# Vanlightly/vsr-tlaplus

Measured on AMD Instinct MI355X. Metric: distinct states/sec (whole node) + time-to-first-violation, VSR 3-replica, higher is better.
Workload: dtype u64

## Files before the change

### vsr_tlaplus_amd/csrc/host_checker.hpp

```cpp
#pragma once

struct PassDst {
  u64* words = nullptr;
  u64 words_cap = 0;
  u64* off = nullptr;
  u64* fp = nullptr;
  u64 cap = 0;
  bool own_words = true;
  bool own_index = true;
};
struct DeepLevelRec { u64 n_new = 0, n_local = 0, generated = 0, max_bag = 0, frontier = 0; };
struct vsrmc_deep_attach;
struct vsrmc_checker {
  vsrmc_model model;
  vsrmc_options opt;
  hipStream_t stream = nullptr;
  hipEvent_t ev[4] = {nullptr, nullptr, nullptr, nullptr};
  Slot* table = nullptr;
  u64 tmask = 0;
  u64* words[2] = {nullptr, nullptr};
  u64* off[2] = {nullptr, nullptr};
  u64* lvl_fp = nullptr;
  u64* pending = nullptr;
  LevelCtl* ctl = nullptr;
// ... 182 lines not shown
    if (hipFuncGetAttributes(&at, c->plain5_kernel) == hipSuccess && dyn + at.sharedSizeBytes <= LDS5_MAX &&
        hipOccupancyMaxActiveBlocksPerMultiprocessor(&nb5, c->plain5_kernel, blk, dyn) == hipSuccess && nb5 >= VSR_OCC + 1) {
      f.kernel = c->plain5_kernel; f.ccap = cc5; f.lds = dyn; f.blocks_per_cu = (unsigned)(VSR_OCC + 1);
    }
  }
  return f;
}

int wset_ensure(vsrmc_checker* c) {
  if (c->opt.world <= 1) return 0;
  if (c->d_wset) {
    if (c->wset_dirty) {
      HIPCHK(hipMemsetAsync(c->h_wset.fp, 0, (c->h_wset.mask + 1) * 8, c->stream));
      HIPCHK(hipMemsetAsync(c->h_wset.epoch, 0, (c->h_wset.mask + 1) * 4, c->stream));
      c->wset_dirty = false;
      c->wepoch = 0;
    }
    return 0;
  }
  u64 slots = std::max<u64>((u64)1 << 12, (c->tmask + 1) / 2);
  while (true) {
    hipError_t e = hipMalloc((void**)&c->h_wset.fp, slots * 8);
    if (e == hipSuccess) e = hipMalloc((void**)&c->h_wset.epoch, slots * 4);
    if (e == hipSuccess) break;
    (void)hipGetLastError();
    if (c->h_wset.fp) (void)hipFree(c->h_wset.fp);
    c->h_wset.fp = nullptr;
    if (slots <= ((u64)1 << 16)) return fail(VSRMC_E_HIP, "hipMalloc of the winner set of the sharded deep search failed");
    slots /= 2;
  }
  c->h_wset.mask = slots - 1;
  HIPCHK(hipMemsetAsync(c->h_wset.fp, 0, slots * 8, c->stream));
  HIPCHK(hipMemsetAsync(c->h_wset.epoch, 0, slots * 4, c->stream));
  HIPCHK(hipMalloc((void**)&c->d_wset, sizeof(WSet)));
  HIPCHK(hipMemcpyAsync(c->d_wset, &c->h_wset, sizeof(WSet), hipMemcpyHostToDevice, c->stream));
  HIPCHK(hipStreamSynchronize(c->stream));
  c->wepoch = 0;
  c->wset_dirty = false;
  return 0;
}
u64 wset_count(const vsrmc_checker* c) {
  u64 n = 0;
  for (const DeepLevelRec& d : c->deep_lv) n += d.n_local;
  return n;
}
int wset_grow(vsrmc_checker* c) {
  if (!c->d_wset) return 1;
  const u64 old_slots = c->h_wset.mask + 1, slots = old_slots * 2;
  u64* nfp = nullptr;
  u32* nep = nullptr;
  u32* d_err = nullptr;
  size_t free_b = 0, total_b = 0;
  if (hipMemGetInfo(&free_b, &total_b) != hipSuccess || (double)slots * 12.0 + 1.0e9 > (double)free_b) return 1;
  bool ok = hipMalloc((void**)&nfp, slots * 8) == hipSuccess && hipMalloc((void**)&nep, slots * 4) == hipSuccess && hipMalloc((void**)&d_err, 4) == hipSuccess;
  ok = ok && hipMemsetAsync(nfp, 0, slots * 8, c->stream) == hipSuccess && hipMemsetAsync(nep, 0, slots * 4, c->stream) == hipSuccess &&
       hipMemsetAsync(d_err, 0, 4, c->stream) == hipSuccess;
  u32 err = 0;
  if (ok) {
    hipLaunchKernelGGL(k_wset_rehash, dim3(4096), dim3(256), 0, c->stream, (const u64*)c->h_wset.fp, (const u32*)c->h_wset.epoch, old_slots, nfp, nep, slots - 1, d_err);
    ok = hipGetLastError() == hipSuccess && hipMemcpyAsync(&err, d_err, 4, hipMemcpyDeviceToHost, c->stream) == hipSuccess && hipStreamSynchronize(c->stream) == hipSuccess && err == 0;
  }
  if (d_err) (void)hipFree(d_err);
  if (!ok) {
    (void)hipGetLastError();
    if (nfp) (void)hipFree(nfp);
    if (nep) (void)hipFree(nep);
    return 1;
  }
  (void)hipFree(c->h_wset.fp);
  (void)hipFree(c->h_wset.epoch);
  c->h_wset.fp = nfp; c->h_wset.epoch = nep; c->h_wset.mask = slots - 1;
  if (hipMemcpy(c->d_wset, &c->h_wset, sizeof(WSet), hipMemcpyHostToDevice) != hipSuccess) return fail(VSRMC_E_HIP, "winner set: descriptor copy");
  return 0;
}
void wset_free(vsrmc_checker* c) {
  if (c->h_wset.fp) (void)hipFree(c->h_wset.fp);
  if (c->h_wset.epoch) (void)hipFree(c->h_wset.epoch);
  if (c->d_wset) (void)hipFree(c->d_wset);
  c->h_wset.fp = nullptr; c->h_wset.epoch = nullptr; c->h_wset.mask = 0; c->d_wset = nullptr; c->wepoch = 0;
}

void deep_free_scratch(vsrmc_checker* c);

int checker_seed(vsrmc_checker* c) {
  const Model& M = c->model.M;
  deep_free_scratch(c);
#ifdef VSRMC_TEST_HOOKS
  c->test_seed_index.clear(); c->test_seed_words.clear(); c->test_seed_off.clear();
#endif
  c->rebase_off = false;
  c->saw_violation = false;
  c->deep = 0;
  c->deep_lv.clear();
  c->deep_g = 2;
  c->deep_distinct = c->deep_generated = 0;
  c->deep_regen_done = false;
  c->hist_new[0] = c->hist_new[1] = 0;
  c->g_last = 16;
  c->cur_rec_w = 0;
  c->failed = 0;
  c->failed_code = 0;
  c->full_recoverable = false;
  HIPCHK(hipSetDevice(c->opt.device));
  if (c->claim_bits) { (void)hipFree(c->claim_bits); c->claim_bits = nullptr; c->claim_w = c->claim_parents = 0; }
  if (c->d_wset && c->wset_used) c->wset_dirty = true;
  c->wset_used = false;
  hipLaunchKernelGGL(k_table_init, dim3(4096), dim3(256), 0, c->stream, c->table, c->tmask + 1);
  HIPCHK(hipGetLastError());
  std::vector<u64> wire, dev(512);
  init_record_wire(M, wire);
  int len = wire_to_device(M, wire.data(), dev.data());
  u64 H[6];
  hash_full_host(M, (const u64*)dev.data(), H);
  for (int i = 0; i < M.np; i++) dev[M.h0 + i] = H[i];
  u64 zero = (u64)len, init_fp = 0;
  u32 init_ak = 0;
  canonical_fp(M, dev[0], &dev[M.h0], &init_fp, &init_ak);
  const bool mine = true;
  if (c->filter) HIPCHK(hipMemsetAsync(c->filter, 0, (c->fmask + 1) * 8, c->stream));
  HIPCHK(hipMemsetAsync(c->ctl, 0, sizeof(LevelCtl), c->stream));
  if (mine) {
    HIPCHK(hipMemcpyAsync(c->words[0], dev.data(), len * 8, hipMemcpyDefault, c->stream));
    HIPCHK(hipMemcpyAsync(c->off[0], &zero, 8, hipMemcpyHostToDevice, c->stream));
    hipLaunchKernelGGL(k_seed, dim3(1), dim3(64), 0, c->stream, M, c->words[0], c->table, c->tmask, c->lvl_fp, c->ctl);
    HIPCHK(hipGetLastError());
  }
  HIPCHK(hipStreamSynchronize(c->stream));
  c->cur = 0;
  c->level = 1;
  c->n_frontier = mine ? 1 : 0;
  c->n_valid = c->n_frontier;
  c->cur_w = (u64)len;
  c->distinct = mine ? 1 : 0;
  c->total_generated = 0;
  c->failed = 0;
  c->cur_max_bag = 0;
  c->bag_known = true;
  c->failed_code = 0;
  c->probe_fp = 0;
  c->probe_level = 0;
  c->probe_extra_fp = 0;
  c->probe_viol.clear();
  c->probe_viol_key.clear();
  c->probe_viol_level = 0;
  deep_attach_restart(c);
  return 0;
}
}

extern "C" {

void vsrmc_options_default(vsrmc_options* o) {
  if (!o) return;
  std::memset(o, 0, sizeof(*o));
  o->device = 0;
  o->table_log2 = 26;
  o->frontier_words = (uint64_t)1 << 27;
  o->frontier_states = (uint64_t)1 << 22;
  o->pending_entries = (uint64_t)1 << 23;
  o->keep_trace = 1;
  o->trace_entries = 0;
  o->rank = 0;
  o->world = 1;
}

static int autosize_options(vsrmc_options* o, const Model& M) {
  if (o->table_log2 != 0 && o->frontier_words != 0) {
    if (o->pending_entries == 0) o->pending_entries = o->exact_ties ? (u64)1 << 24 : (u64)1 << 16;
    if (o->frontier_states == 0) o->frontier_states = std::max<u64>((u64)1 << 16, o->frontier_words / 24);
    return 0;
  }
  size_t free_b = 0, total_b = 0;
  HIPCHK(hipSetDevice(o->device));
  HIPCHK(hipMemGetInfo(&free_b, &total_b));
  const char* share_env = std::getenv("VSRMC_AUTOSIZE_SHARE");
  const double share = share_env ? std::max(1.0, std::atof(share_env)) : 1.0;
  double avail = ((double)free_b - 4.0e9) / share;
  if (avail < 256e6) return fail(VSRMC_E_HIP, "less than 256 MB of free device memory to size the checker from");
  if (o->table_log2 == 0) {
    int lg = 8;
    while (lg < 36 && (double)((u64)1 << (lg + 1)) * 16.0 <= 0.30 * avail) lg++;
    o->table_log2 = lg;
  }
  avail -= (double)((u64)1 << o->table_log2) * 16.0;
  if (o->world > 1 && !o->exact_ties) avail -= (double)((u64)1 << (o->filter_log2 > 0 ? o->filter_log2 : o->table_log2)) * 8.0;
  if (o->world > 1 && !o->exact_ties) avail -= (double)((u64)1 << o->table_log2) * 6.0;
  if (o->pending_entries == 0) o->pending_entries = o->exact_ties ? (u64)1 << 24 : (u64)1 << 16;
// ... 671 lines not shown
```

### vsr_tlaplus_amd/csrc/vsr_deep.hpp

```cpp
#pragma once

namespace {

typedef DeepLevelRec DeepLevel;

struct Slicer {
  u64 cap_n, cap_w, g1, stride;
  u64 cap_c = ~(u64)0;
  double yield_n = 0, yield_w = 0;
  u64 worst() const {
    const u64 sz = std::min<u64>(std::min<u64>(cap_n / (4 * g1), cap_w / (4 * g1 * stride)), cap_c);
    return std::max<u64>(128, sz & ~(u64)127);
  }
  u64 next() const {
    if (yield_n <= 0) return worst();
    const double sz = std::min((double)cap_n / (3.0 * std::max(yield_n, 1e-3)), (double)cap_w / (3.0 * std::max(yield_w, 1e-3)));
    return std::max<u64>(worst(), std::min<u64>(cap_c, std::max<u64>(128, (u64)std::min(sz, 1e15) & ~(u64)127)));
  }
  void expect(double per_n, double per_w) { yield_n = std::max(yield_n, per_n); yield_w = std::max(yield_w, per_w); }
  void observe(u64 n_src, u64 n_out, u64 w_out) {
    if (!n_src) return;
    yield_n = std::max(yield_n, (double)n_out / (double)n_src);
    yield_w = std::max(yield_w, (double)w_out / (double)n_src);
  }
};

struct DeepRun;
struct DeepIo {
  void* ctx = nullptr;
  int world = 1;
  u64 cand_cap = 0;
  int (*pass)(void* ctx, const u64* sw, const u64* so, u64 n, u64 p_off, int level, int mode, u64 bag, const PassDst* dst) = nullptr;
  int (*any)(void* ctx, u64* flag) = nullptr;
  int (*reduce)(void* ctx, DeepRun* R) = nullptr;
  int (*resolve)(void* ctx, DeepRun* R) = nullptr;
};

struct DeepRun {
  vsrmc_checker* c;
  const DeepIo* io = nullptr;
  int base;
  int last_regen;
  bool insert;
  vsrmc_level_info ins, prb;
  u64 viol_ins = ~(u64)0;
  u32 mask_ins = 0, mask_prb = 0;
  std::vector<u64> bad;
  u64 launches = 0, n_slices = 0, n_subs = 0;
  u64* d_sum = nullptr;
  bool rebase = false;
  u64* d_cnt = nullptr;
  u32* d_err = nullptr;
  int err = 0;
  int probed_level() const { return last_regen + (insert ? 2 : 1); }
};

void deep_free_scratch(vsrmc_checker* c) {
  for (PassDst& B : c->scratch) {
    if (B.words && B.own_words) (void)hipFree(B.words);
    if (B.off && B.own_index) (void)hipFree(B.off);
    if (B.fp && B.own_index) (void)hipFree(B.fp);
  }
  c->scratch.clear();
  c->scratch0 = PassDst();
  c->scratch_carved = false;
  c->scratch_buf = -1;
  c->scratch_front = 0;
}

int deep_plan_scratch(vsrmc_checker* c, int count, bool carve = true, u64 front = 0) {
  if (count < 0) count = 0;
  if (count > 400) return fail(VSRMC_E_REP, "deep search: more than 400 nested levels");
  const int nxt = c->cur ^ 1;
  if ((c->host_frontier >> nxt) & 1) carve = false;
  front = (front + 63) & ~(u64)63;
  const bool same_buf = !c->scratch_carved || c->scratch_buf == nxt;
  if ((size_t)count <= c->scratch.size() && c->scratch_front == front && same_buf && (c->scratch_carved == carve || (count == 0 && !carve))) return 0;
  deep_free_scratch(c);
  if (count == 0) return 0;
  size_t free_b = 0, total_b = 0;
  HIPCHK(hipMemGetInfo(&free_b, &total_b));
  const char* share_env = std::getenv("VSRMC_AUTOSIZE_SHARE");
  const double share = share_env ? std::max(1.0, std::atof(share_env)) : 1.0;
  const double reserve = std::max(0.0, (double)free_b - 1.0e9) / share;
  if (front >= c->words_cap(nxt)) carve = false;
  const double idle_w = (double)(c->words_cap(nxt) - (carve ? front : 0));
  const int with0 = front ? 0 : 1;
  const u64 floor_w = (u64)1 << 21;
  const double w_old = std::max((double)floor_w, std::min(idle_w / 4.0, reserve / (double)count / 9.34));
  const double cost_old = (with0 ? 1.0 / idle_w : 0.0) + (double)count / w_old;
  int best_n = 0;
  double best_s = 0;
  if (carve)
    for (int n_idle = 1; n_idle <= count + with0; n_idle++) {
      const double from_res = (double)(count + with0 - n_idle) * 9.34 + (double)(n_idle - with0) * 1.34;
      const double s = std::min(idle_w / (double)n_idle, from_res > 0 ? reserve / from_res : 1e30);
      if (s > best_s) { best_s = s; best_n = n_idle; }
    }
  const bool carved = carve && best_n >= 1 + with0 && best_s >= (double)floor_w && (double)(count + with0) / best_s < cost_old;
  const u64 wcap = carved ? (u64)best_s & ~(u64)63 : (u64)w_old;
  auto alloc_index = [&](PassDst& B) -> bool {
    B.cap = std::max<u64>((u64)1 << 15, B.words_cap / 12);
    return hipMalloc((void**)&B.off, (B.cap + 1) * 8) == hipSuccess && hipMalloc((void**)&B.fp, B.cap * 8) == hipSuccess;
  };
  bool ok = true;
  if (carved && with0) {
    c->scratch0.words = c->words[nxt]; c->scratch0.words_cap = wcap; c->scratch0.own_words = false;
    c->scratch0.off = c->off[nxt]; c->scratch0.fp = c->lvl_fp; c->scratch0.own_index = false;
    c->scratch0.cap = std::min<u64>(c->opt.frontier_states, std::max<u64>((u64)1 << 15, wcap / 12));
  }
  for (int k = 1; k <= count && ok; k++) {
    PassDst B;
    B.words_cap = wcap;
    if (carved && k - 1 + with0 < best_n) { B.words = c->words[nxt] + front + (u64)(k - 1 + with0) * wcap; B.own_words = false; }
    else ok = hipMalloc((void**)&B.words, B.words_cap * 8) == hipSuccess;
    ok = ok && alloc_index(B);
    c->scratch.push_back(B);
  }
  if (!ok) {
    (void)hipGetLastError();
    deep_free_scratch(c);
    return fail(VSRMC_E_HIP, "hipMalloc of a deep-search scratch buffer failed");
  }
  c->scratch_carved = carve;
  c->scratch_buf = nxt;
  c->scratch_front = front;
  return 0;
}

int deep_buffer(vsrmc_checker* c, int k, PassDst* out) {
  const int nxt = c->cur ^ 1;
  if (k == 0) {
// ... 39 lines not shown
  u64 f = (mine ? 1 : 0) | (R.err ? 2 : 0);
  if (R.io) *rc = R.io->any(R.io->ctx, &f);
  if (!*rc && f >= 2) *rc = R.err ? R.err : fail(VSRMC_E_STATE, "deep pass: another rank failed between two exchanges");
  return !*rc && (f & 1) != 0;
}
int deep_local_fail(DeepRun& R, int rc) {
  if (!R.io) return rc;
  if (!R.err) R.err = rc;
  return 0;
}
u64 deep_cand_bound(const DeepRun& R, u64 g1) {
  if (!R.io || R.io->world <= 1) return ~(u64)0;
  return std::max<u64>(128, (u64)(0.45 * (double)R.io->cand_cap * (double)R.io->world / (double)std::max<u64>(1, g1)) & ~(u64)127);
}

int deep_probe(DeepRun& R, const PassDst& B, u64 n, int lv, u64 bag) {
  vsrmc_checker* c = R.c;
  if (!n) return 0;
  c->expand_ms = 0;
  if (R.err) return 0;
  int rc = expand_pass(c, B.words, B.off, n, 0, lv + 1, MODE_PROBE, bag);
  R.launches += c->extra_launches;
  if (!rc && c->h.limit_unchecked) {
    R.prb.limit_rechecked += c->h.limit_unchecked;
    c->probe_all_actions = true;
    rc = expand_pass(c, B.words, B.off, n, 0, lv + 1, MODE_PROBE, bag);
    c->probe_all_actions = false;
    R.launches += 1 + c->extra_launches;
  }
  if (rc) return deep_local_fail(R, rc);
  R.launches++;
  deep_acc(&R.prb, c->h, c->expand_ms);
  if (c->h.n_pending) {
    R.mask_prb |= c->h.viol_mask;
    if (c->h.n_pending > c->opt.pending_entries || R.bad.size() / 2 + c->h.n_pending > ((u64)1 << 24))
      return deep_local_fail(R, fail(VSRMC_E_REP, "more violating successors in the probed level than the pending list holds (pending_entries)"));
    const size_t at = R.bad.size();
    R.bad.resize(at + 2 * c->h.n_pending);
    if (hipMemcpy(R.bad.data() + at, c->pending, 16 * c->h.n_pending, hipMemcpyDeviceToHost) != hipSuccess)
      return deep_local_fail(R, fail(VSRMC_E_HIP, "deep search: copy of the probe's candidates"));
  }
  return 0;
}

int deep_export(DeepRun& R, const PassDst& B, u64 part) {
  vsrmc_checker* c = R.c;
  if (!part) return 0;
  const int nxt = c->cur ^ 1;
  hipLaunchKernelGGL(k_export, dim3((unsigned)((part + 63) / 64)), dim3(64), 0, c->stream, (const u64*)B.words, B.off, B.fp, (u64)0, part,
                     c->words[nxt], c->scratch_front ? c->scratch_front : c->words_cap(nxt), c->off[nxt], c->lvl_fp, c->opt.frontier_states, R.d_cnt, R.d_err);
  if (hipGetLastError() != hipSuccess || hipStreamSynchronize(c->stream) != hipSuccess) return fail(VSRMC_E_HIP, "deep search: k_export (re-basing)");
  return 0;
}

int deep_descend(DeepRun& R, const u64* src_words, const u64* src_off, u64 n_idx, u64 src_bag, int lv, int k) {
  vsrmc_checker* c = R.c;
  const Model& M = c->model.M;
  PassDst B;
  int rc = deep_buffer(c, k, &B);
  if (rc) return rc;
  Slicer sl;
  sl.cap_n = B.cap; sl.cap_w = B.words_cap; sl.g1 = std::max<u64>(1, c->deep_g); sl.stride = (u64)c->lds_stride;
  sl.cap_c = deep_cand_bound(R, sl.g1);
  const bool regen = lv + 1 <= R.last_regen;
  const DeepLevel& next = c->deep_lv[(size_t)(lv - R.base)];
  if (regen) {
    const u64 parents = lv == R.base ? c->n_valid : c->deep_lv[(size_t)(lv - R.base - 1)].n_local;
    const double per_n = (double)next.n_local / (double)std::max<u64>(1, parents);
    const double wbar = (lv == R.base ? (double)c->cur_w / (double)std::max<u64>(1, c->n_valid) : (double)(M.fixed + (int)src_bag)) + 2.0;
    sl.expect(per_n, per_n * wbar);
  }
  const u64 out_bag = regen ? std::min<u64>(next.max_bag, (u64)M.max_bag) : 0;
  for (u64 a = 0; deep_more(R, a < n_idx, &rc);) {
    if (rc) return rc;
    const u64 n = a < n_idx ? std::min<u64>(sl.next(), n_idx - a) : 0;
    c->expand_ms = 0;
    rc = deep_run_pass(R, src_words, src_off + a, n, (R.io && c->opt.world > 1) ? 0 : a, lv + 1, regen ? MODE_REGEN : MODE_NORMAL, src_bag, &B);
    if (rc) return rc;
    if (n) R.launches += 1 + c->extra_launches;
    a += n;
    if (n) (k == 0 ? R.n_slices : R.n_subs)++;
    const u64 part = c->h.n_new;
    sl.observe(n, part, c->h.words_new);
    if (regen) {
      R.ins.materialize_ms += c->expand_ms;
      if (c->deep_attach && !R.io && (rc = deep_where_slice(c, B, part, lv + 1, 0, out_bag, false)) != 0) return rc;
      if (lv + 1 == R.last_regen && !R.insert) rc = R.rebase ? deep_export(R, B, part) : deep_probe(R, B, part, lv + 1, out_bag);
      else rc = deep_descend(R, B.words, B.off, part, out_bag, lv + 1, k + 1);
      if (rc) return rc;
      continue;
    }
    deep_acc(&R.ins, c->h, c->expand_ms);
    R.ins.record_words += c->h.rec_words;
    R.ins.max_bag = std::max<u64>(R.ins.max_bag, c->h.max_bag);
    if (c->h.viol_fp != ~(u64)0) {
      R.mask_ins |= c->h.viol_mask;
      R.viol_ins = std::min<u64>(R.viol_ins, c->h.viol_fp);
    }
    if (!part) continue;
    const u64 bag_new = std::min<u64>(c->h.max_bag, (u64)M.max_bag);
    {
      u64 hsum[3] = {0, 0, 0};
      bool ok = hipMemsetAsync(R.d_sum, 0, 24, c->stream) == hipSuccess;
      if (ok) hipLaunchKernelGGL(k_level_checksum, dim3(1024), dim3(256), 0, c->stream, B.fp, part, R.d_sum);
      ok = ok && hipGetLastError() == hipSuccess && hipMemcpyAsync(hsum, R.d_sum, 24, hipMemcpyDeviceToHost, c->stream) == hipSuccess &&
           hipStreamSynchronize(c->stream) == hipSuccess;
      if (!ok) {
        rc = deep_local_fail(R, fail(VSRMC_E_HIP, "deep search: k_level_checksum"));
        if (rc) return rc;
        continue;
      }
      R.ins.fp_xor ^= hsum[0];
      R.ins.fp_sum += hsum[1];
      R.ins.n_new += hsum[2];
    }
    if (c->deep_attach && !R.io && (rc = deep_where_slice(c, B, part, lv + 1, 1, bag_new, R.viol_ins == ~(u64)0)) != 0) return rc;
    if (R.viol_ins != ~(u64)0) continue;
    rc = deep_probe(R, B, part, lv + 1, bag_new);
    if (rc) return rc;
  }
  return rc;
}

int deep_resolve(DeepRun& R) {
  vsrmc_checker* c = R.c;
  const u64 nbad = R.bad.size() / 2;
  if (!nbad) return 0;
  const int plevel = R.probed_level();
  std::vector<std::pair<u64, u64>> pairs(nbad);
  for (u64 i = 0; i < nbad; i++) pairs[i] = std::make_pair(R.bad[2 * i], R.bad[2 * i + 1]);
  std::sort(pairs.begin(), pairs.end());
  std::vector<u64> fps;
  for (u64 i = 0; i < nbad; i++)
    if (i == 0 || pairs[i].first != pairs[i - 1].first) fps.push_back(pairs[i].first);
  std::vector<uint8_t> seen8(fps.size(), 0);
  int rc = vsrmc_checker_seen_batch(c, fps.data(), (u64)fps.size(), plevel, seen8.data());
  if (rc) return rc;
  u64 first = ~(u64)0, key = ~(u64)0;
  size_t g = 0;
  for (u64 i = 0; i < nbad; i++) {
    if (i && pairs[i].first != pairs[i - 1].first) g++;
    if (seen8[g]) continue;
    R.prb.pending++;
    if (first == ~(u64)0) { first = pairs[i].first; key = pairs[i].second; }
    if (c->probe_viol.empty() || c->probe_viol.back() != pairs[i].first) {
      c->probe_viol.push_back(pairs[i].first);
      c->probe_viol_key.push_back(pairs[i].second);
    }
  }
  c->probe_viol_level = plevel;
  if (first == ~(u64)0) return 0;
  int found = 0;
  u64 pfp = 0, pmeta = 0;
  rc = table_lookup(c, meta_pfp(key), plevel - 1, 1, &found, &pfp, &pmeta);
  if (rc) return rc;
  if (found > 1) return fail(VSRMC_E_STATE, "ambiguous predecessor pointer: several states of the parent's level share the 45 fingerprint bits the violating successor keeps of its parent");
  R.prb.viol_fp = first;
  R.prb.viol_mask = (int32_t)R.mask_prb;
  if (found) { c->probe_fp = pfp; c->probe_level = plevel - 1; c->probe_extra_fp = first; }
  return 0;
}

int deep_check_ready(vsrmc_checker* c, int extra_levels, bool sharded) {
  if (c->opt.exact_ties) return fail(VSRMC_E_STATE, "levels beyond the record buffers need a single-pass checker");
  if (!sharded && c->opt.world > 1) return fail(VSRMC_E_STATE, "a sharded checker goes beyond its record buffers with vsrmc_shard_loop_deepen");
  if (c->failed) return fail(VSRMC_E_STATE, "the checker stopped on an error");
  if (c->level + c->deep + extra_levels >= 511) return fail(VSRMC_E_REP, "more than 510 BFS levels");
  return 0;
}

int deep_first_pass(vsrmc_checker* c, vsrmc_level_info* ins, const DeepIo* io = nullptr) {
  const Model& M = c->model.M;
  DeepRun R;
  R.c = c; R.io = io; R.base = c->level; R.last_regen = c->level; R.insert = true;
  std::memset(&R.ins, 0, sizeof(R.ins));
  std::memset(&R.prb, 0, sizeof(R.prb));
  R.ins.viol_fp = R.ins.viol_index = R.prb.viol_fp = R.prb.viol_index = ~(u64)0;
  const double t0 = now_s();
  const u64 bagL = c->bag_known ? c->cur_max_bag : (u64)M.max_bag;
  c->deep = 1;
  c->deep_lv.assign(1, DeepLevel());
  const u64 cb = deep_cand_bound(R, std::max<u64>(c->deep_g, c->g_last));
  if (!io || c->opt.world == 1) deep_claim_bits_alloc(c, bagL);
  int rc = 0;
  for (u64 a = 0; deep_more(R, a < c->n_frontier, &rc);) {
    if (rc) break;
    const u64 n = a < c->n_frontier ? std::min<u64>(cb, c->n_frontier - a) : 0;
    c->expand_ms = 0;
    rc = deep_run_pass(R, c->words[c->cur], c->off[c->cur] + a, n, (io && c->opt.world > 1) ? 0 : a, c->level + 1, MODE_INSERT, bagL, nullptr);
    if (rc) break;
    a += n;
    if (n) R.launches += 1 + c->extra_launches;
    deep_acc(&R.ins, c->h, c->expand_ms);
    R.ins.n_new += c->h.n_new;
    R.ins.max_bag = std::max<u64>(R.ins.max_bag, c->h.max_bag);
    R.ins.fp_xor ^= c->h.fp_xor;
    R.ins.fp_sum += c->h.fp_sum;
    if (c->h.viol_fp != ~(u64)0) { R.mask_ins |= c->h.viol_mask; R.viol_ins = std::min<u64>(R.viol_ins, c->h.viol_fp); }
  }
  if (rc) { c->failed = 1; return rc; }
  const u64 n_local = R.ins.n_new, frontier_local = c->n_valid;
  R.ins.frontier = c->n_valid;
  R.ins.viol_fp = R.viol_ins;
  R.ins.viol_mask = (int32_t)R.mask_ins;
  if (io && (rc = io->reduce(io->ctx, &R)) != 0) { c->failed = 1; return rc; }
  DeepLevel& d = c->deep_lv[0];
  d.n_new = R.ins.n_new; d.n_local = n_local; d.generated = R.ins.generated; d.max_bag = R.ins.max_bag; d.frontier = R.ins.frontier;
  c->deep_g = std::max<u64>(c->deep_g, (R.ins.generated + R.ins.frontier - 1) / std::max<u64>(1, R.ins.frontier) + 1);
  (void)frontier_local;
  *ins = R.ins;
  ins->level = c->level + (R.ins.n_new ? 1 : 0);
  if (R.ins.n_new == 0) { c->deep = 0; c->deep_lv.clear(); }
  ins->pending = R.launches;
  c->deep_distinct = c->distinct + (io ? n_local : R.ins.n_new);
  c->deep_generated = c->total_generated + R.ins.generated;
  ins->distinct = c->deep_distinct;
  ins->total_generated = c->deep_generated;
  ins->seconds = now_s() - t0;
  ins->viol_index = ~(u64)0;
  if (ins->viol_fp != ~(u64)0) {
    c->probe_fp = ins->viol_fp;
    c->probe_level = c->level + 1;
    c->probe_extra_fp = 0;
  } else {
    ins->viol_mask = 0;
  }
  return 0;
}

int deep_pass(vsrmc_checker* c, int last_regen, bool insert, vsrmc_level_info* ins, vsrmc_level_info* prb, const DeepIo* io = nullptr) {
  const Model& M = c->model.M;
  DeepRun R;
  R.c = c; R.io = io; R.base = c->level; R.last_regen = last_regen; R.insert = insert;
  std::memset(&R.ins, 0, sizeof(R.ins));
  std::memset(&R.prb, 0, sizeof(R.prb));
  R.ins.viol_fp = R.ins.viol_index = R.prb.viol_fp = R.prb.viol_index = ~(u64)0;
  const double t0 = now_s();
  if (io && c->opt.world > 1) {
    c->wepoch++;
  } else if (c->deep_regen_done) {
    hipLaunchKernelGGL(k_table_untake, dim3(4096), dim3(256), 0, c->stream, c->table, c->tmask + 1, c->level + 1);
    HIPCHK(hipGetLastError());
    HIPCHK(hipStreamSynchronize(c->stream));
  }
  c->deep_regen_done = true;
  int rc = 0;
  if (hipMalloc((void**)&R.d_sum, 24) != hipSuccess) { (void)hipGetLastError(); R.d_sum = nullptr; rc = fail(VSRMC_E_HIP, "deep pass: hipMalloc of the checksum words"); }
  struct FreeSum { u64* p; ~FreeSum() { if (p) (void)hipFree(p); } } free_sum{R.d_sum};
  if (insert) { c->deep_lv.resize((size_t)(last_regen + 1 - c->level)); c->deep_lv.back() = DeepLevel(); }
  if (!rc) rc = deep_plan_scratch(c, last_regen - c->level - (insert ? 0 : 1));
  if (io) {
    u64 bad_plan = rc ? 1 : 0;
    const int arc = io->any(io->ctx, &bad_plan);
    if (!rc && (arc || bad_plan)) rc = arc ? arc : fail(VSRMC_E_HIP, "deep pass: another rank could not allocate its scratch buffers");
  }
  if (rc) { c->failed = 1; return rc; }
  if (io) { u64 sync = 0; rc = io->any(io->ctx, &sync); }
  const bool scan = c->deep_attach && !io;
  if (!rc && scan) rc = deep_where_begin(c, last_regen + (insert ? 1 : 0));
  if (!rc) rc = deep_descend(R, c->words[c->cur], c->off[c->cur], c->n_frontier, c->bag_known ? c->cur_max_bag : (u64)M.max_bag, c->level, 0);
  if (scan) rc = deep_where_end(c, rc);
  if (rc) { c->failed = 1; return rc; }
  const u64 n_local = R.ins.n_new;
  R.ins.viol_fp = R.viol_ins;
  R.ins.viol_mask = (int32_t)R.mask_ins;
  R.prb.viol_mask = (int32_t)R.mask_prb;
  if (io && (rc = io->reduce(io->ctx, &R)) != 0) { c->failed = 1; return rc; }
  const double dt = now_s() - t0;
  const DeepLevel& below = c->deep_lv[(size_t)(last_regen - c->level - 1)];
  if (insert) {
    DeepLevel& d = c->deep_lv.back();
    d.n_new = R.ins.n_new; d.n_local = n_local; d.generated = R.ins.generated; d.max_bag = R.ins.max_bag; d.frontier = below.n_new;
    c->deep_g = std::max<u64>(c->deep_g, (R.ins.generated + below.n_new - 1) / std::max<u64>(1, below.n_new) + 1);
    c->deep_distinct += io ? n_local : R.ins.n_new;
    c->deep_generated += R.ins.generated;
    *ins = R.ins;
    ins->level = last_regen + (R.ins.n_new ? 1 : 0);
    ins->frontier = below.n_new;
    ins->distinct = c->deep_distinct;
    ins->total_generated = c->deep_generated;
    ins->pending = R.launches;
    ins->words_new = (R.n_slices << 32) | (R.n_subs & 0xFFFFFFFFull);
    ins->viol_index = ~(u64)0;
    const double ms_all = R.ins.expand_ms + R.ins.materialize_ms + R.prb.expand_ms;
    ins->seconds = dt * ((R.ins.expand_ms + R.ins.materialize_ms) / std::max(1e-9, ms_all));
    if (R.ins.n_new) c->deep = last_regen + 1 - c->level;
    else c->deep_lv.pop_back();
    if (ins->viol_fp != ~(u64)0) {
      c->probe_fp = ins->viol_fp;
      c->probe_level = last_regen + 1;
      c->probe_extra_fp = 0;
      return 0;
    }
    ins->viol_mask = 0;
  }
  R.prb.level = R.probed_level();
  R.prb.frontier = insert ? R.ins.n_new : below.n_new;
  R.prb.distinct = c->deep_distinct;
  R.prb.total_generated = c->deep_generated + R.prb.generated;
  R.prb.seconds = insert ? dt - ins->seconds : dt;
  R.prb.viol_fp = R.prb.viol_index = ~(u64)0;
  R.prb.viol_mask = 0;
  if (!insert) {
    R.prb.record_words = R.ins.record_words;
    R.prb.materialize_ms = R.ins.materialize_ms;
    R.prb.words_new = (R.n_slices << 32) | (R.n_subs & 0xFFFFFFFFull);
  }
  rc = io ? io->resolve(io->ctx, &R) : deep_resolve(R);
  if (rc) return rc;
  *prb = R.prb;
  return 0;
}

bool rebase_pays(const vsrmc_checker* c) {
  if (!c->deep || c->failed || c->opt.world > 1 || c->opt.exact_ties || c->rebase_off) return false;
  const DeepLevel& top = c->deep_lv.back();
  if (top.n_new == 0) return false;
  if (!(c->deep >= 2 || top.n_new <= c->n_valid)) return false;
  const Model& M = c->model.M;
  const int nxt = c->cur ^ 1;
  const double words = (double)top.n_new * (double)(M.fixed + (int)std::min<u64>(top.max_bag, (u64)M.max_bag));
  return words <= 0.8 * (double)c->words_cap(nxt) && (double)top.n_new <= 0.8 * (double)c->opt.frontier_states;
}

int deep_rebase(vsrmc_checker* c, vsrmc_level_info* out) {
  const Model& M = c->model.M;
  const int K = c->level + c->deep;
  DeepRun R;
  R.c = c; R.base = c->level; R.last_regen = K; R.insert = false; R.rebase = true;
  std::memset(&R.ins, 0, sizeof(R.ins));
  std::memset(&R.prb, 0, sizeof(R.prb));
  R.ins.viol_fp = R.ins.viol_index = R.prb.viol_fp = R.prb.viol_index = ~(u64)0;
  const double t0 = now_s();
  const u64 front_w = c->deep_lv.back().n_new * (u64)(M.fixed + (int)std::min<u64>(c->deep_lv.back().max_bag, (u64)M.max_bag));
  int rc = deep_plan_scratch(c, c->deep, true, front_w);
  if (rc) { c->rebase_off = true; return 1; }
  struct FreeCnt { u64* p; u32* q; ~FreeCnt() { if (p) (void)hipFree(p); if (q) (void)hipFree(q); } } free_cnt{nullptr, nullptr};
  if (hipMalloc((void**)&R.d_cnt, 16) != hipSuccess) { (void)hipGetLastError(); R.d_cnt = nullptr; c->rebase_off = true; return 1; }
  free_cnt.p = R.d_cnt;
  if (hipMalloc((void**)&R.d_err, 4) != hipSuccess) { (void)hipGetLastError(); R.d_err = nullptr; c->rebase_off = true; return 1; }
  free_cnt.q = R.d_err;
  if (hipMemsetAsync(R.d_cnt, 0, 16, c->stream) != hipSuccess || hipMemsetAsync(R.d_err, 0, 4, c->stream) != hipSuccess) { (void)hipGetLastError(); c->rebase_off = true; return 1; }
  if (c->deep_regen_done) {
    hipLaunchKernelGGL(k_table_untake, dim3(4096), dim3(256), 0, c->stream, c->table, c->tmask + 1, c->level + 1);
    HIPCHK(hipGetLastError());
    HIPCHK(hipStreamSynchronize(c->stream));
  }
  c->deep_regen_done = true;
  rc = c->deep_attach ? deep_where_begin(c, K) : 0;
  if (!rc) rc = deep_descend(R, c->words[c->cur], c->off[c->cur], c->n_frontier, c->bag_known ? c->cur_max_bag : (u64)M.max_bag, c->level, 1);
  if (c->deep_attach) rc = deep_where_end(c, rc);
  if (rc) { c->failed = 1; return rc; }
  u64 cnt[2] = {0, 0};
  u32 xerr = 0;
  HIPCHK(hipMemcpy(cnt, R.d_cnt, 16, hipMemcpyDeviceToHost));
  HIPCHK(hipMemcpy(&xerr, R.d_err, 4, hipMemcpyDeviceToHost));
  const DeepLevel top = c->deep_lv.back();
  if (xerr || cnt[0] != top.n_new) {
    c->failed = 1;
    return fail(xerr ? VSRMC_E_REP : VSRMC_E_STATE, xerr ? std::string("re-basing: the idle record buffer is too small for the level after all")
                : "re-basing: level " + std::to_string(K) + " has " + std::to_string((unsigned long long)top.n_new) + " states, the descent regenerated " +
                  std::to_string((unsigned long long)cnt[0]));
  }
  const u64 below = c->deep >= 2 ? c->deep_lv[c->deep_lv.size() - 2].n_new : c->n_valid;
  c->cur ^= 1;
  c->level = K;
  c->n_frontier = cnt[0];
  c->n_valid = cnt[0];
  c->cur_w = cnt[1];
  c->cur_rec_w = cnt[1];
  c->distinct = c->deep_distinct;
  c->total_generated = c->deep_generated;
  c->cur_max_bag = std::min<u64>(top.max_bag, (u64)M.max_bag);
  c->bag_known = true;
  c->hist_new[0] = below;
  c->hist_new[1] = top.n_new;
  c->g_last = (top.generated + std::max<u64>(1, top.frontier) - 1) / std::max<u64>(1, top.frontier) + 1;
  c->deep = 0;
  c->deep_lv.clear();
  if (c->claim_bits) { (void)hipFree(c->claim_bits); c->claim_bits = nullptr; c->claim_w = c->claim_parents = 0; }
  c->deep_regen_done = false;
  std::memset(out, 0, sizeof(*out));
  out->level = K;
  out->frontier = below;
  out->n_new = top.n_new;
  out->distinct = c->distinct;
  out->total_generated = c->total_generated;
  out->max_bag = top.max_bag;
  out->words_new = cnt[1];
  out->record_words = cnt[1];
  out->pending = R.launches;
  out->materialize_ms = R.ins.materialize_ms;
  out->seconds = now_s() - t0;
  out->viol_fp = out->viol_index = ~(u64)0;
  return 0;
}

}

extern "C" {

int32_t vsrmc_checker_deepen(vsrmc_checker* c, vsrmc_level_info* inserted, vsrmc_level_info* probed) {
  if (!c || !inserted || !probed) return fail(VSRMC_E_ARG, "NULL argument");
  int rc = deep_check_ready(c, 2, false);
  if (rc) return rc;
  HIPCHK(hipSetDevice(c->opt.device));
  std::memset(inserted, 0, sizeof(*inserted));
  std::memset(probed, 0, sizeof(*probed));
  inserted->viol_fp = inserted->viol_index = probed->viol_fp = probed->viol_index = ~(u64)0;
  c->probe_fp = 0;
  c->probe_level = 0;
  c->probe_extra_fp = 0;
  c->probe_viol.clear();
  c->probe_viol_key.clear();
  c->probe_viol_level = 0;
  if (c->deep == 0) return deep_first_pass(c, inserted);
  return deep_pass(c, c->level + c->deep, true, inserted, probed);
}

int32_t vsrmc_checker_probe2(vsrmc_checker* c, vsrmc_level_info* virt, vsrmc_level_info* probe) {
  if (!c || !virt || !probe) return fail(VSRMC_E_ARG, "NULL argument");
  if (c->deep) return fail(VSRMC_E_STATE, "vsrmc_checker_probe2 starts from a materialised level");
  if (c->deep_attach) return fail(VSRMC_E_STATE, "vsrmc_checker_probe2: predicates are attached (vsrmc_checker_deep_attach): they are evaluated by vsrmc_checker_deepen / _advance");
  vsrmc_level_info none;
  int rc = vsrmc_checker_deepen(c, virt, probe);
  if (rc || virt->viol_mask || virt->n_new == 0) return rc;
  rc = deep_pass(c, c->level + 1, false, &none, probe);
  return rc;
}

int32_t vsrmc_checker_probe3(vsrmc_checker* c, vsrmc_level_info* virt1, vsrmc_level_info* virt2, vsrmc_level_info* probe) {
  if (!c || !virt1 || !virt2 || !probe) return fail(VSRMC_E_ARG, "NULL argument");
  if (c->deep) return fail(VSRMC_E_STATE, "vsrmc_checker_probe3 starts from a materialised level");
  if (c->deep_attach) return fail(VSRMC_E_STATE, "vsrmc_checker_probe3: predicates are attached (vsrmc_checker_deep_attach): they are evaluated by vsrmc_checker_deepen / _advance");
  std::memset(virt2, 0, sizeof(*virt2));
  virt2->viol_fp = virt2->viol_index = ~(u64)0;
  int rc = vsrmc_checker_deepen(c, virt1, probe);
  if (rc || virt1->viol_mask || virt1->n_new == 0) return rc;
  return vsrmc_checker_deepen(c, virt2, probe);
}

}
```

### vsr_tlaplus_amd/csrc/vsr_kernels.hpp

```cpp
#pragma once
#include <hip/hip_runtime.h>

#include "vsr_actions.hpp"
#include "vrst_actions.hpp"
#include "vras_actions.hpp"

namespace vsr {

template <int MODEL>
struct ModelOps;
template <>
struct ModelOps<0> {
  template <bool GUARD_ONLY, typename PTR>
  static VSR_HD bool gen_(const Model& M, PTR rec, int ord, Delta& D) { return gen<GUARD_ONLY>(M, rec, ord, D); }
  template <typename PTR>
  static VSR_HD u32 guard_pre(const Model& M, PTR rec, u64 hdr, const u64* Areg, int slot, int* kind0, int info) {
    return guard_slot_pre(M, rec, hdr, Areg, slot, kind0, info);
  }
  template <typename PTR>
  static VSR_HD u32 guard(const Model& M, PTR rec, int slot, int* kind0) { return guard_slot(M, rec, slot, kind0); }
  static VSR_HD int other_kind(int) { return A_SendGetState; }
  template <typename PTR>
  static VSR_HD void hash_child_(const Model& M, PTR rec, const Delta& D, u64* Hc) { hash_child(M, rec, D, Hc); }
  template <typename PTR>
// ... 1235 lines not shown
    u64 idx;
    bool overflow = false;
    if (idx_left < (u32)nwin) {
      u64 nb = 0;
      if (lane == 0) nb = atomicAdd((unsigned long long*)cnt_n, (unsigned long long)ichunk);
      nb = readlane64(nb, 0);
      if (nb + ichunk > nx_cap) overflow = true;
      idx = rank < idx_left ? idx_base + rank : nb + (rank - idx_left);
      idx_base = nb + ((u32)nwin - idx_left);
      idx_left = ichunk - ((u32)nwin - idx_left);
    } else {
      idx = idx_base + rank;
      idx_base += (u32)nwin;
      idx_left -= (u32)nwin;
    }
    if (w_left < total) {
      u64 nb = 0;
      if (lane == 0) nb = atomicAdd((unsigned long long*)cnt_w, (unsigned long long)wchunk);
      nb = readlane64(nb, 0);
      if (nb + wchunk > nx_words_cap) overflow = true;
      w_base = nb;
      w_left = wchunk;
    }
    const u64 dst = w_base + (u64)(incl - clen);
    rec_words += total;
    w_base += total;
    w_left -= total;
    if (overflow) {
      if (lane == 0) raise_error(ctl, ERR_FRONTIER_FULL, idx_base);
      idx_left = 0;
      w_left = 0;
      continue;
    }
    for (int g = 0; g < 64; g += VSR_MAT_GROUP) {
      if (((wmask >> g) & ((1u << VSR_MAT_GROUP) - 1)) == 0) continue;
#pragma unroll
      for (int q = 0; q < VSR_MAT_GROUP; q++) {
        const u64 d = readlane64(dst, g + q);
        const int n = __builtin_amdgcn_readlane(clen, g + q);
        if (lane < n) nx_words[d + lane] = s_slot[(g + q) * stride + lane];
        if (lane + 64 < n) nx_words[d + lane + 64] = s_slot[(g + q) * stride + lane + 64];
      }
    }
    if (win) {
      nx_off[idx] = (dst << 8) | (u64)clen;
      lvl_fp[idx] = fp;
      if (bad) {
        atomicMin((unsigned long long*)&ctl->viol_fp, (unsigned long long)fp);
        atomicOr(&ctl->viol_mask, (u32)bad);
      }
    }
    int mb = nbag;
    for (int o = 32; o > 0; o >>= 1) {
      int t = __shfl_down(mb, o);
      mb = t > mb ? t : mb;
    }
    if (lane == 0 && (u64)mb > __hip_atomic_load(&ctl->max_bag, __ATOMIC_RELAXED, __HIP_MEMORY_SCOPE_AGENT))
      atomicMax((unsigned long long*)&ctl->max_bag, (unsigned long long)mb);
    lds_wave_sync();
    cyc_write += __builtin_readcyclecounter() - c_3;
  }
  if (lane == 0) {
    atomicAdd((unsigned long long*)&ctl->phase_cycles[5], (unsigned long long)(cyc_fetch + cyc_stage));
    atomicAdd((unsigned long long*)&ctl->phase_cycles[6], (unsigned long long)cyc_gen);
    atomicAdd((unsigned long long*)&ctl->phase_cycles[7], (unsigned long long)cyc_write);
    atomicAdd((unsigned long long*)&ctl->rec_words, (unsigned long long)rec_words);
  }
  for (u32 k = lane; k < idx_left; k += 64) {
    nx_off[idx_base + k] = 0;
    lvl_fp[idx_base + k] = 0;
  }
}

__global__ void k_count_valid(const u64* __restrict__ refs, u64 n, u64* out) {
  u64 i = (u64)blockIdx.x * blockDim.x + threadIdx.x;
  const u64 stride = (u64)gridDim.x * blockDim.x;
  u32 c = 0;
  for (; i < n; i += stride) c += refs[i] != 0 ? 1 : 0;
  for (int o = 32; o > 0; o >>= 1) c += __shfl_down(c, o);
  if ((threadIdx.x & 63) == 0 && c) atomicAdd((unsigned long long*)out, (unsigned long long)c);
}

__global__ void k_level_checksum(const u64* __restrict__ fps, u64 n, u64* out) {
  u64 i = (u64)blockIdx.x * blockDim.x + threadIdx.x;
  const u64 stride = (u64)gridDim.x * blockDim.x;
  u64 x = 0, s = 0, c = 0;
  for (; i < n; i += stride) {
    const u64 f = fps[i];
    x ^= f;
    s += f;
    c += f != 0 ? 1 : 0;
  }
  for (int o = 32; o > 0; o >>= 1) {
    x ^= __shfl_down(x, o);
    s += __shfl_down(s, o);
    c += __shfl_down(c, o);
  }
  if ((threadIdx.x & 63) == 0) {
    if (x) atomicXor((unsigned long long*)&out[0], (unsigned long long)x);
    if (s) atomicAdd((unsigned long long*)&out[1], (unsigned long long)s);
    if (c) atomicAdd((unsigned long long*)&out[2], (unsigned long long)c);
  }
}

__global__ void k_table_level_checksum(const Slot* __restrict__ table, u64 n_slots, int level, u64* out) {
  u64 i = (u64)blockIdx.x * blockDim.x + threadIdx.x;
  const u64 stride = (u64)gridDim.x * blockDim.x;
  u64 x = 0, s = 0, c = 0;
  for (; i < n_slots; i += stride) {
    const u64 f = table[i].fp;
    if (f != 0 && meta_level(table[i].meta) == level) { x ^= f; s += f; c++; }
  }
  for (int o = 32; o > 0; o >>= 1) {
    x ^= __shfl_down(x, o);
    s += __shfl_down(s, o);
    c += __shfl_down(c, o);
  }
  if ((threadIdx.x & 63) == 0 && c) {
    atomicXor((unsigned long long*)&out[0], (unsigned long long)x);
    atomicAdd((unsigned long long*)&out[1], (unsigned long long)s);
    atomicAdd((unsigned long long*)&out[2], (unsigned long long)c);
  }
}

__global__ void k_table_rehash(const Slot* __restrict__ old_table, u64 n_old, Slot* table, u64 tmask, u32* err) {
  u64 i = (u64)blockIdx.x * blockDim.x + threadIdx.x;
  const u64 stride = (u64)gridDim.x * blockDim.x;
  for (; i < n_old; i += stride) {
    const Slot s = old_table[i];
    if (s.fp == 0) continue;
    u32 np = 0;
    const Probe p = probe_insert(table, tmask, s.fp, CntReg{&np});
    if (p.full) { atomicExch(err, (u32)ERR_TABLE_FULL); continue; }
    table[p.slot].meta = s.meta;
  }
}

__global__ void k_wset_rehash(const u64* __restrict__ old_fp, const u32* __restrict__ old_epoch, u64 n_old, u64* fp, u32* epoch, u64 mask, u32* err) {
  u64 i = (u64)blockIdx.x * blockDim.x + threadIdx.x;
  const u64 stride = (u64)gridDim.x * blockDim.x;
  for (; i < n_old; i += stride) {
    const u64 f = old_fp[i];
    if (f == 0) continue;
    u64 j = wset_home(f, mask);
    bool done = false;
    for (u64 step = 0; step <= mask && step < 65536 && !done; step++, j = (j + 1) & mask)
      if (atomicCAS((unsigned long long*)&fp[j], 0ull, (unsigned long long)f) == 0) { epoch[j] = old_epoch[i]; done = true; }
    if (!done) atomicExch(err, (u32)ERR_TABLE_FULL);
  }
}

__global__ void k_table_untake(Slot* table, u64 n_slots, int min_level) {
  u64 i = (u64)blockIdx.x * blockDim.x + threadIdx.x;
  const u64 stride = (u64)gridDim.x * blockDim.x;
  for (; i < n_slots; i += stride) {
    const u64 m = table[i].meta;
    if (table[i].fp != 0 && (m & META_TAKEN) && m != META_EMPTY && meta_level(m) >= min_level) table[i].meta = m & ~META_TAKEN;
  }
}

__global__ void k_table_init(Slot* table, u64 slots) {
  for (u64 i = (u64)blockIdx.x * blockDim.x + threadIdx.x; i < slots; i += (u64)gridDim.x * blockDim.x) {
    table[i].fp = 0;
    table[i].meta = META_EMPTY;
  }
}

__global__ void k_claim_batch(Slot* table, u64 tmask, const u64* __restrict__ entries, u64 n, int level, u64* rslot,
                              LevelCtl* ctl) {
  u64 i = (u64)blockIdx.x * blockDim.x + threadIdx.x;
  if (i >= n) return;
  bool found_old, full;
  u32 np = 0;
  u64 slot = table_claim(table, tmask, entries[2 * i], entries[2 * i + 1], level, &found_old, CntReg{&np}, &full);
  if (full) raise_error(ctl, ERR_TABLE_FULL, entries[2 * i]);
  rslot[i] = found_old ? ~(u64)0 : slot;
  atomicAdd((unsigned long long*)&ctl->probes, (unsigned long long)np);
}
__global__ void k_verdict(Slot* table, const u64* __restrict__ entries, const u64* __restrict__ rslot, u64 n, uint8_t* verdict) {
  u64 i = (u64)blockIdx.x * blockDim.x + threadIdx.x;
  if (i >= n) return;
// ... 560 lines not shown
```

Before: 1.839 billion.

## Defer deep-search checksum readback to one fetch per pass and vectorize checksum kernel

In the non-distributed deep search, each slice's checksum kernel now accumulates into a device buffer without a per-slice memset, device-to-host copy and stream synchronize. The totals are read back once after the descent finishes. The checksum kernel now uses 128-bit loads with four-way unrolling, reduces across waves in shared memory so each block issues one set of atomics, and launches half as many blocks. Optional phase-clock instrumentation is also added behind a compile flag; it synchronizes the stream when enabled. Reading the counts once at the end means n_new is no longer updated per slice, so any code inside the loop that relied on the running total would see stale values.

```diff
diff --git a/vsr_tlaplus_amd/csrc/host_checker.hpp b/vsr_tlaplus_amd/csrc/host_checker.hpp
--- a/vsr_tlaplus_amd/csrc/host_checker.hpp
+++ b/vsr_tlaplus_amd/csrc/host_checker.hpp
@@ -288,9 +288,30 @@
 
 void deep_free_scratch(vsrmc_checker* c);
 
+#if VSR_PHASE_CLOCKS
+struct DeepClocks {
+  u64 pc[2][9];
+  u64 launches[2];
+  double kernel_ms[2];
+  double sum_s, claim_alloc_s, claim_free_s, plan_s, unplan_s;
+  u64 n_sum, n_claim_alloc, n_claim_free, n_plan, n_unplan;
+};
+static DeepClocks g_deep_clk = {};
+struct DeepClockScope {
+  hipStream_t s; double* acc; u64* n; double t0;
+  DeepClockScope(hipStream_t s_, double* acc_, u64* n_) : s(s_), acc(acc_), n(n_) { (void)hipStreamSynchronize(s); t0 = now_s(); }
+  ~DeepClockScope() { (void)hipStreamSynchronize(s); *acc += now_s() - t0; ++*n; }
+};
+#endif
+
 int checker_seed(vsrmc_checker* c) {
   const Model& M = c->model.M;
-  deep_free_scratch(c);
+  {
+#if VSR_PHASE_CLOCKS
+    DeepClockScope clk_unplan(c->stream, &g_deep_clk.unplan_s, &g_deep_clk.n_unplan);
+#endif
+    deep_free_scratch(c);
+  }
 #ifdef VSRMC_TEST_HOOKS
   c->test_seed_index.clear(); c->test_seed_words.clear(); c->test_seed_off.clear();
 #endif
@@ -308,7 +329,12 @@
   c->failed_code = 0;
   c->full_recoverable = false;
   HIPCHK(hipSetDevice(c->opt.device));
-  if (c->claim_bits) { (void)hipFree(c->claim_bits); c->claim_bits = nullptr; c->claim_w = c->claim_parents = 0; }
+  {
+#if VSR_PHASE_CLOCKS
+    DeepClockScope clk_free(c->stream, &g_deep_clk.claim_free_s, &g_deep_clk.n_claim_free);
+#endif
+    if (c->claim_bits) { (void)hipFree(c->claim_bits); c->claim_bits = nullptr; c->claim_w = c->claim_parents = 0; }
+  }
   if (c->d_wset && c->wset_used) c->wset_dirty = true;
   c->wset_used = false;
   hipLaunchKernelGGL(k_table_init, dim3(4096), dim3(256), 0, c->stream, c->table, c->tmask + 1);
diff --git a/vsr_tlaplus_amd/csrc/vsr_deep.hpp b/vsr_tlaplus_amd/csrc/vsr_deep.hpp
--- a/vsr_tlaplus_amd/csrc/vsr_deep.hpp
+++ b/vsr_tlaplus_amd/csrc/vsr_deep.hpp
@@ -48,6 +48,7 @@
   std::vector<u64> bad;
   u64 launches = 0, n_slices = 0, n_subs = 0;
   u64* d_sum = nullptr;
+  bool sum_queued = false;
   bool rebase = false;
   u64* d_cnt = nullptr;
   u32* d_err = nullptr;
@@ -253,6 +254,15 @@
     if (n) (k == 0 ? R.n_slices : R.n_subs)++;
     const u64 part = c->h.n_new;
     sl.observe(n, part, c->h.words_new);
+#if VSR_PHASE_CLOCKS
+    if (n) {
+      const int kd = regen ? 0 : 1;
+      for (int a = 0; a < 8; a++) g_deep_clk.pc[kd][a] += c->h.phase_cycles[a];
+      g_deep_clk.pc[kd][8] += c->h.act_generated[0];
+      g_deep_clk.launches[kd]++;
+      g_deep_clk.kernel_ms[kd] += c->expand_ms;
+    }
+#endif
     if (regen) {
       R.ins.materialize_ms += c->expand_ms;
       if (c->deep_attach && !R.io && (rc = deep_where_slice(c, B, part, lv + 1, 0, out_bag, false)) != 0) return rc;
@@ -271,9 +281,17 @@
     if (!part) continue;
     const u64 bag_new = std::min<u64>(c->h.max_bag, (u64)M.max_bag);
     {
+#if VSR_PHASE_CLOCKS
+      DeepClockScope clk_sum(c->stream, &g_deep_clk.sum_s, &g_deep_clk.n_sum);
+#endif
+      if (!R.io) {
+        hipLaunchKernelGGL(k_level_checksum, dim3(512), dim3(256), 0, c->stream, B.fp, part, R.d_sum);
+        if (hipGetLastError() != hipSuccess) return fail(VSRMC_E_HIP, "deep search: k_level_checksum");
+        R.sum_queued = true;
+      } else {
       u64 hsum[3] = {0, 0, 0};
       bool ok = hipMemsetAsync(R.d_sum, 0, 24, c->stream) == hipSuccess;
-      if (ok) hipLaunchKernelGGL(k_level_checksum, dim3(1024), dim3(256), 0, c->stream, B.fp, part, R.d_sum);
+      if (ok) hipLaunchKernelGGL(k_level_checksum, dim3(512), dim3(256), 0, c->stream, B.fp, part, R.d_sum);
       ok = ok && hipGetLastError() == hipSuccess && hipMemcpyAsync(hsum, R.d_sum, 24, hipMemcpyDeviceToHost, c->stream) == hipSuccess &&
            hipStreamSynchronize(c->stream) == hipSuccess;
       if (!ok) {
@@ -284,6 +302,7 @@
       R.ins.fp_xor ^= hsum[0];
       R.ins.fp_sum += hsum[1];
       R.ins.n_new += hsum[2];
+      }
     }
     if (c->deep_attach && !R.io && (rc = deep_where_slice(c, B, part, lv + 1, 1, bag_new, R.viol_ins == ~(u64)0)) != 0) return rc;
     if (R.viol_ins != ~(u64)0) continue;
@@ -291,6 +310,18 @@
     if (rc) return rc;
   }
   return rc;
+}
+
+int deep_sum_fetch(DeepRun& R) {
+  if (!R.sum_queued) return 0;
+  u64 hsum[3] = {0, 0, 0};
+  if (hipMemcpyAsync(hsum, R.d_sum, 24, hipMemcpyDeviceToHost, R.c->stream) != hipSuccess || hipStreamSynchronize(R.c->stream) != hipSuccess)
+    return fail(VSRMC_E_HIP, "deep search: k_level_checksum");
+  R.ins.fp_xor ^= hsum[0];
+  R.ins.fp_sum += hsum[1];
+  R.ins.n_new += hsum[2];
+  R.sum_queued = false;
+  return 0;
 }
 
 int deep_resolve(DeepRun& R) {
@@ -352,7 +383,12 @@
   c->deep = 1;
   c->deep_lv.assign(1, DeepLevel());
   const u64 cb = deep_cand_bound(R, std::max<u64>(c->deep_g, c->g_last));
-  if (!io || c->opt.world == 1) deep_claim_bits_alloc(c, bagL);
+  if (!io || c->opt.world == 1) {
+#if VSR_PHASE_CLOCKS
+    DeepClockScope clk_alloc(c->stream, &g_deep_clk.claim_alloc_s, &g_deep_clk.n_claim_alloc);
+#endif
+    deep_claim_bits_alloc(c, bagL);
+  }
   int rc = 0;
   for (u64 a = 0; deep_more(R, a < c->n_frontier, &rc);) {
     if (rc) break;
@@ -418,8 +454,14 @@
   int rc = 0;
   if (hipMalloc((void**)&R.d_sum, 24) != hipSuccess) { (void)hipGetLastError(); R.d_sum = nullptr; rc = fail(VSRMC_E_HIP, "deep pass: hipMalloc of the checksum words"); }
   struct FreeSum { u64* p; ~FreeSum() { if (p) (void)hipFree(p); } } free_sum{R.d_sum};
+  if (!rc && hipMemsetAsync(R.d_sum, 0, 24, c->stream) != hipSuccess) rc = fail(VSRMC_E_HIP, "deep pass: the checksum words");
   if (insert) { c->deep_lv.resize((size_t)(last_regen + 1 - c->level)); c->deep_lv.back() = DeepLevel(); }
-  if (!rc) rc = deep_plan_scratch(c, last_regen - c->level - (insert ? 0 : 1));
+  {
+#if VSR_PHASE_CLOCKS
+    DeepClockScope clk_plan(c->stream, &g_deep_clk.plan_s, &g_deep_clk.n_plan);
+#endif
+    if (!rc) rc = deep_plan_scratch(c, last_regen - c->level - (insert ? 0 : 1));
+  }
   if (io) {
     u64 bad_plan = rc ? 1 : 0;
     const int arc = io->any(io->ctx, &bad_plan);
@@ -430,6 +472,7 @@
   const bool scan = c->deep_attach && !io;
   if (!rc && scan) rc = deep_where_begin(c, last_regen + (insert ? 1 : 0));
   if (!rc) rc = deep_descend(R, c->words[c->cur], c->off[c->cur], c->n_frontier, c->bag_known ? c->cur_max_bag : (u64)M.max_bag, c->level, 0);
+  if (!rc) rc = deep_sum_fetch(R);
   if (scan) rc = deep_where_end(c, rc);
   if (rc) { c->failed = 1; return rc; }
   const u64 n_local = R.ins.n_new;
@@ -571,6 +614,24 @@
 
 extern "C" {
 
+#if VSR_PHASE_CLOCKS
+int32_t vsrmc_deep_clocks(double* out, int32_t cap) {
+  const DeepClocks& k = g_deep_clk;
+  std::vector<double> v;
+  for (int kd = 0; kd < 2; kd++) {
+    for (int a = 0; a < 9; a++) v.push_back((double)k.pc[kd][a]);
+    v.push_back((double)k.launches[kd]);
+    v.push_back(k.kernel_ms[kd]);
+  }
+  const double host[10] = {k.sum_s, (double)k.n_sum, k.claim_alloc_s, (double)k.n_claim_alloc, k.claim_free_s, (double)k.n_claim_free,
+                           k.plan_s, (double)k.n_plan, k.unplan_s, (double)k.n_unplan};
+  v.insert(v.end(), host, host + 10);
+  int32_t n = 0;
+  for (; n < cap && n < (int32_t)v.size(); n++) out[n] = v[(size_t)n];
+  return n;
+}
+#endif
+
 int32_t vsrmc_checker_deepen(vsrmc_checker* c, vsrmc_level_info* inserted, vsrmc_level_info* probed) {
   if (!c || !inserted || !probed) return fail(VSRMC_E_ARG, "NULL argument");
   int rc = deep_check_ready(c, 2, false);
diff --git a/vsr_tlaplus_amd/csrc/vsr_kernels.hpp b/vsr_tlaplus_amd/csrc/vsr_kernels.hpp
--- a/vsr_tlaplus_amd/csrc/vsr_kernels.hpp
+++ b/vsr_tlaplus_amd/csrc/vsr_kernels.hpp
@@ -1341,21 +1341,38 @@
 }
 
 __global__ void k_level_checksum(const u64* __restrict__ fps, u64 n, u64* out) {
-  u64 i = (u64)blockIdx.x * blockDim.x + threadIdx.x;
-  const u64 stride = (u64)gridDim.x * blockDim.x;
+  typedef u64 u64x2 __attribute__((ext_vector_type(2)));
+  __shared__ u64 s_red[16][3];
+  const u64 t = (u64)blockIdx.x * blockDim.x + threadIdx.x;
+  const u64 nthr = (u64)gridDim.x * blockDim.x;
   u64 x = 0, s = 0, c = 0;
-  for (; i < n; i += stride) {
-    const u64 f = fps[i];
-    x ^= f;
-    s += f;
-    c += f != 0 ? 1 : 0;
+  auto acc = [&](u64 f) { x ^= f; s += f; c += f != 0 ? 1 : 0; };
+  const u64 head = (n > 0 && ((uintptr_t)fps & 8)) ? 1 : 0;
+  const u64 pairs = (n - head) / 2;
+  const u64x2* v = (const u64x2*)(fps + head);
+  u64 i = t;
+  for (; i + 3 * nthr < pairs; i += 4 * nthr) {
+    const u64x2 a0 = v[i], a1 = v[i + nthr], a2 = v[i + 2 * nthr], a3 = v[i + 3 * nthr];
+    acc(a0.x); acc(a0.y); acc(a1.x); acc(a1.y); acc(a2.x); acc(a2.y); acc(a3.x); acc(a3.y);
+  }
+  for (; i < pairs; i += nthr) {
+    const u64x2 a0 = v[i];
+    acc(a0.x); acc(a0.y);
+  }
+  if (t == 0) {
+    if (head) acc(fps[0]);
+    if ((n - head) & 1) acc(fps[n - 1]);
   }
   for (int o = 32; o > 0; o >>= 1) {
     x ^= __shfl_down(x, o);
     s += __shfl_down(s, o);
     c += __shfl_down(c, o);
   }
-  if ((threadIdx.x & 63) == 0) {
+  const int wave = (int)(threadIdx.x >> 6), nwaves = (int)((blockDim.x + 63) >> 6);
+  if ((threadIdx.x & 63) == 0) { s_red[wave][0] = x; s_red[wave][1] = s; s_red[wave][2] = c; }
+  __syncthreads();
+  if (threadIdx.x == 0) {
+    for (int w = 1; w < nwaves; w++) { x ^= s_red[w][0]; s += s_red[w][1]; c += s_red[w][2]; }
     if (x) atomicXor((unsigned long long*)&out[0], (unsigned long long)x);
     if (s) atomicAdd((unsigned long long*)&out[1], (unsigned long long)s);
     if (c) atomicAdd((unsigned long long*)&out[2], (unsigned long long)c);
```

Result: no change. 1.851 billion (median of 6 runs) (+0.7%).
